# evolbioinfo/pastml

Hardware: AMD Instinct MI355X
Metric: ACR nodes*states*chars/sec (full marginal pass: P(t) + bottom-up + top-down + posteriors) (higher is better)
Workload: dtype f64; 1 GPU; BASELINE config 4 shard: balanced tree, 1048576 tips (2097151 nodes), k=64 states, F81, 32 characters per GPU (32 in total), marginal (BU+TD+posteriors); tips=1048576, nodes=2097151, states=64, chars_per_gpu=32, chars_total=32, substitution_model=F81, collective=local

## Files before the change

pastml_amd/csrc/pml_api.hip:

```cpp
#define PML_PLAIN_KERNELS
#include "pml_launch.h"
#include "pml_kernels_counts.h"
#include "pml_kernels_eigen_gemm.h"
#include "pml_comm.h"
#include "pml_pij_window.h"

#ifndef PML_BUILD_DIGEST
#define PML_BUILD_DIGEST "unknown"
#endif
static const char kBuildDigest[] = "PML_BUILD_DIGEST=" PML_BUILD_DIGEST;

static thread_local std::string g_last_error;

int pml_fail(int code, const char* fmt, ...) {
    char buf[1024];
    va_list ap;
    va_start(ap, fmt);
    vsnprintf(buf, sizeof(buf), fmt, ap);
    va_end(ap);
    g_last_error = buf;
    return code;
}

template <typename T>
// ... 973 lines not shown

static PmlSweepTraits sweep_traits(const pml_ctx* ctx) {
    PmlSweepTraits t;
    t.f81 = ctx->kind == PML_MODEL_F81;
    t.eigen_fused = eigen_fused(ctx);
    t.eigen_gemm = eigen_gemm(ctx);
    t.eigen_joint_valu = eigen_joint_valu(ctx);
    t.hky_fused = hky_fused(ctx);
    t.wide_states = wide_states(ctx);
    t.k = ctx->k;
    t.W = ctx->W;
    t.C = ctx->C;
    t.sched_cols = ctx->sched_cols;
    t.n_roots = ctx->n_roots;
    t.n_cherries = ctx->n_cherries;
    t.has_init = ctx->has_init;
    t.fuse = ctx->fuse;
    t.Gf = ctx->cols.Gf;
    t.Gt = ctx->cols.Gt;
    t.bu_wide_lanes = ctx->cols.bu_wide_lanes;
    t.level_lists_sorted = ctx->cols.level_lists_sorted;
    t.single_launch = single_launch_sweeps(ctx);
    t.blocks = block_schedule(ctx);
    t.super = super_sweeps(ctx);
    t.thin = thin_bottom_up(ctx);
    t.deep = deep_top_down(ctx);
    t.narrow_units = (int)ctx->tune.get(T_NARROW_UNITS, 0);
    t.no_td_tail = ctx->tune.on(T_NO_TD_TAIL);
    t.no_eigg_tiers = ctx->tune.on(T_NO_EIGG_TIERS);
    t.no_spin_wait = ctx->tune.on(T_NO_SPIN_WAIT);
    t.waves = PML_WAVES_PER_BLOCK;
    const int ks4 = (ctx->k + 3) / 4;
    t.eig_nb = ks4 % 4 == 0 ? 1 : (ks4 % 2 == 0 ? 2 : 4);
    return t;
}

static PmlSchedules schedules_of(const pml_ctx* ctx) {
    return {&ctx->blocks, &ctx->thin, &ctx->deep, &ctx->sup, &ctx->eig_tiers, &ctx->bt_tiers, &ctx->bu_level_vec_f,
            &ctx->bu_level_vec, &ctx->td_cherry_prefix};
}

static int run_plan(pml_ctx* ctx, const std::vector<PmlLaunch>& whole_plan, bool bottom_up, int is_marginal, bool force_prep) {
    const bool windowed = ctx->pij_window > 0 && ctx->kind == PML_MODEL_EIGEN;
    const int wtab = bottom_up ? 0 : 1;
    const std::vector<PmlWindowStep>* cached = nullptr;
    std::vector<PmlLaunch> cut;
    if (windowed) {
        auto same = [](const PmlLaunch& a, const PmlLaunch& b) {
            return a.op == b.op && a.list == b.list && a.kind == b.kind && a.bracket == b.bracket && a.branch == b.branch &&
                   a.signal == b.signal && a.cherries == b.cherries && a.first == b.first && a.count == b.count && a.arg == b.arg;
        };
        for (const pml_ctx::WindowCut& c : ctx->win_cuts)
            if (c.plan.size() == whole_plan.size() && std::equal(c.plan.begin(), c.plan.end(), whole_plan.begin(), same)) cached = &c.steps;
        if (cached == nullptr) {
            PmlWindowPlan W;
            const std::string bad = pml_plan_pij_window(whole_plan, ctx->forest, ctx->bu_order, ctx->td_parents, ctx->pij_window, W);
            if (!bad.empty()) return fail(PML_ERR_INVALID, "%s", bad.c_str());
            if (!W.branches.empty() && W.branches != ctx->win_branches[wtab])
                return fail(PML_ERR_INVALID, "the sweep's runs are not the ones the window's branch lists were uploaded for");
            if (ctx->win_cuts.size() >= 16) ctx->win_cuts.clear();
            ctx->win_cuts.push_back(pml_ctx::WindowCut{whole_plan, std::move(W.steps)});
            cached = &ctx->win_cuts.back().steps;
        }
        cut.reserve(cached->size());
        for (const PmlWindowStep& w : *cached) cut.push_back(w.launch);
    }
    static const std::vector<PmlWindowStep> no_steps;
    const std::vector<PmlWindowStep>& steps = windowed ? *cached : no_steps;
    const std::vector<PmlLaunch>& plan = windowed ? cut : whole_plan;
    size_t at = 0;
    const pml_ctx::EigenTiers& E = ctx->eig_tiers;
    const pml_ctx::BacktraceTiers& B = ctx->bt_tiers;
    const int* order = bottom_up ? ctx->d_bu_order : nullptr;
    const int* offsets = bottom_up ? ctx->d_bu_offsets : ctx->d_td_offsets;
    const int gemm_mode = bottom_up ? PML_EIGG_BU : PML_EIGG_TD;
    const int eig_mode = !bottom_up ? PML_EIG_TD : (is_marginal ? PML_EIG_BU_MARG : PML_EIG_BU_JOINT);
    int open = PML_NO_BRACKET;
    long long launches = 0;
    for (const PmlLaunch& r : plan) {
        if (ctx->tune.on(T_DEBUG))
            fprintf(stderr, "pml plan: branch %d op %d list %d kind %d first %d count %d arg %d bracket %d signal %d\n", r.branch,
                    r.op, r.list, r.kind, r.first, r.count, r.arg, r.bracket, (int)r.signal);
        if (r.bracket != open) {
            if (open != PML_NO_BRACKET) PML_TRY(prof_end(ctx, open, launches));
            if (r.bracket != PML_NO_BRACKET) PML_TRY(prof_begin(ctx));
            open = r.bracket;
            launches = 0;
        }
        ++launches;
        const PmlWindowStep* run = windowed ? &steps[at] : nullptr;
        ++at;
        if (run != nullptr && run->build_count > 0) {
            PML_TRY(launch_pij_wide_list(ctx, ctx->d_pij_window, ctx->pij_window, ctx->d_win_branches[wtab] + run->build_first,
                                         run->build_count));
            ++launches;
        }
        const bool joint = r.kind == EIG_JOINT, gemm = r.kind == EIG_GEMM;
        switch (r.op) {
            case OP_RESET_ERR:
                hipLaunchKernelGGL(reset_err_kernel, dim3((ctx->C + 63) / 64), dim3(64), 0, ctx->stream, ctx->d_err, ctx->C,
                                   r.arg ? ctx->d_tip_rest_count : nullptr);
                HIP_TRY(hipGetLastError());
                break;
            case OP_PREP:
                if (!windowed) PML_TRY(run_prep(ctx, force_prep, true));
                break;
            case OP_LOGLIK:
                hipLaunchKernelGGL(loglik_kernel, dim3((ctx->C + PML_BLOCK - 1) / PML_BLOCK), dim3(PML_BLOCK), 0, ctx->stream,
                                   tree_of(ctx), cols_of(ctx, true), state_of(ctx), ctx->C, is_marginal ? 1 : 0, ctx->h_loglik,
                                   ctx->h_err);
                HIP_TRY(hipGetLastError());
                break;
            case OP_LEVEL:
                PML_TRY(dispatch_sweep(ctx, (SweepKind)r.kind, r.list, r.first, r.count, r.cherries, bottom_up,
                                       windowed && (r.list == L_BU_PLAIN || r.list == L_TD_PLAIN) ? wtab : -1));
                break;
            case OP_ROOTS:
                PML_TRY(dispatch_sweep(ctx, SW_ROOTS, L_NONE, 0, r.count));
                break;
            case OP_LEVELS: {
                const bool whole = r.list == L_BU_FUSED || r.list == L_TD_FUSED;
                const int do_prep = (bottom_up && r.arg && (ctx->results.pij_stale() || force_prep)) ? 1 : 0;
                PML_TRY(dispatch_small_f81(ctx, bottom_up, r.signal, do_prep, whole ? r.first : 0, r.count,
                                           whole ? nullptr : ctx->d_unit_lists[r.list], whole ? nullptr : ctx->d_list_offsets[r.list] + r.first,
                                           bottom_up ? 0 : r.arg));
                break;
            }
            case OP_BLOCKS:
                PML_TRY(dispatch_blocks_f81(ctx, bottom_up, r.first, r.signal));
                break;
            case OP_SUPER:
                PML_TRY(dispatch_super_f81(ctx, bottom_up));
                break;
            case OP_STACK:
                PML_TRY(dispatch_stack_f81(ctx, bottom_up, r.first));
                break;
            case OP_EIG_TIPS:
                if (joint) PML_TRY(launch_eigen_joint_tips(ctx));
                else if (gemm) PML_TRY(launch_eigen_gemm(ctx, PML_EIGG_TIPS, ctx->d_tips, 0, ctx->n_tips));
                else PML_TRY(launch_eigen_tips(ctx, is_marginal ? 0 : 1));
                break;
            case OP_EIG_LEVEL: {
                const int* nodes = order ? order + r.first : nullptr;
                const int first = order ? 0 : r.first;
                if (joint) PML_TRY(launch_eigen_joint(ctx, ctx->d_bu_units + r.first, nullptr, 0, r.count));
                else if (gemm) PML_TRY(launch_eigen_gemm(ctx, gemm_mode, nodes, first, r.count));
                else PML_TRY(launch_eigen_fused(ctx, eig_mode, nodes, first, r.count, 0));
                break;
            }
            case OP_EIG_NARROW:
                if (joint) PML_TRY(launch_eigen_joint(ctx, ctx->d_bu_units, offsets, r.first, r.count));
                else if (gemm) PML_TRY(launch_eigen_gemm_narrow(ctx, gemm_mode, order, offsets, r.first, r.count));
                else PML_TRY(launch_eigen_narrow(ctx, eig_mode, order, offsets, r.first, r.count));
                break;
            case OP_EIG_TIER: {
                const pml_ctx::EigenTiers::Tier& T = E.tiers[r.first];
                if (joint) PML_TRY(launch_eigen_joint(ctx, E.d_units, E.d_lv, 0, T.depth, E.d_start + T.first_block, T.n_blocks));
                else PML_TRY(launch_eigen_gemm_narrow(ctx, PML_EIGG_BU, E.d_nodes, E.d_lv, 0, T.depth, E.d_start + T.first_block,
                                                      T.n_blocks));
                break;
            }
            case OP_BT_NARROW:
                hipLaunchKernelGGL(joint_backtrace_narrow_kernel, dim3(1, ctx->C), dim3(PML_BLOCK), 0, ctx->stream,
                                   tree_of(ctx), cols_of(ctx), state_of(ctx), ctx->d_td_offsets, r.first, r.count);
                HIP_TRY(hipGetLastError());
// ... 1457 lines not shown
```

pastml_amd/csrc/pml_kernels_f81.h:

```cpp
#pragma once
#include "pml_device.h"
#include "pml_schedule.h"

typedef unsigned char pml_jt;

struct PmlTree {
    int N;
    int n_roots;
    const int* parent;
    const int* first_child;
    const int* n_children;
    const double* dist;
    const int* post_rank;
    const unsigned char* kind;
};

struct PmlCols {
    int k, ks, W;
    int no_wide_lean;
    const u64* masks;
    const u64* masks_init;
    const double* pi;
    const double* active;
};
// ... 2327 lines not shown
        if (staged) td_stage_flush<G, R>(L, c, S, (stage & 4) != 0);
        cur = nxt;
        idx = nxt_idx;
    }
}


template <int G, int R>
__device__ __forceinline__ void td_f81_super_tips(const LaneCtx<G, R>& L, const PmlCols& c, const double (&prod3)[R],
                                                  i64 le, int cfc, const TipLane& tl, int jx) {
    constexpr int GC = Gather<G>::GC;
    double P3 = 0.0;
    bool have_P3 = false;
#pragma unroll
    for (int q = 0; q < 2; ++q) {
        const int ts = L.group_base + jx * GC + q;
        f81_finish_tip_word<G, R>(L, c, prod3, le, P3, have_P3, cfc + q, __shfl(tl.mask, ts, 64), __shfl(tl.e, ts, 64),
                                  __shfl(tl.s, ts, 64));
    }
}

template <int R>
struct TdSuperLoads {
    double po[R];
    double ls;
    i64 pe;
    double e, s;
    i64 be;
    u64 own;
    ChildLane cl;
    TipLane tl;
};

template <int G, int R>
__device__ __forceinline__ void td_f81_super_issue(const LaneCtx<G, R>& L, const PmlCols& c, const SuperRegs& s, int j,
                                                   TdSuperLoads<R>& ld) {
    const int ch = s.fc + j;
    node_load_vec<G, R>(L, c, L.post, s.n, ld.po);
    ld.ls = L.lhsum[s.n];
    ld.pe = L.lhe[s.n];
    ld.e = L.E[ch];
    ld.s = L.S[ch];
    ld.be = L.be[ch];
    ld.own = L.mask[(unsigned)ch];
    f81_gather_issue<G, R>(L, super_child<G>(s, j, L.g), ld.cl, ld.tl);
}

template <int R>
__device__ __forceinline__ void td_super_loads_arrived(TdSuperLoads<R>& ld) {
#pragma unroll
    for (int r = 0; r < R; ++r) asm volatile("" : "+v"(ld.po[r]));
    asm volatile("" : "+v"(ld.ls), "+v"(ld.pe), "+v"(ld.e), "+v"(ld.s), "+v"(ld.be), "+v"(ld.own));
    asm volatile("" : "+v"(ld.cl.e), "+v"(ld.cl.s), "+v"(ld.cl.mask), "+v"(ld.cl.be), "+v"(ld.tl.e), "+v"(ld.tl.s),
                      "+v"(ld.tl.mask));
}

template <int G, int R, bool LANES, bool PIPE>
__device__ __forceinline__ void td_f81_super_unit(const LaneCtx<G, R>& L, const PmlTree& t, const PmlCols& c,
                                                  const PmlState& st, const SuperRegs& s, int j, TdSuperLoads<R>& in,
                                                  double* ps_row) {
    if (PIPE) td_super_loads_arrived<R>(in);
    const u64 kbits = state_bits(c.k);
    const int ch = s.fc + j;
    const UnitRegs u = super_child<G>(s, j, L.g);
    double prod[R];
    const i64 pe = in.pe;
#pragma unroll
    for (int r = 0; r < R; ++r) prod[r] = in.po[r] * (in.ls * L.ipi_r[r]);
    const double e = in.e;
    const double s_child = in.s;
    const i64 bec = in.be;
    BuLoads<R> ld;
    ld.own = in.own;
// ... 217 lines not shown
    return bu_f81_marg_body<G, R, true, false>(L, t, c, st, un, top);
}

template <int G, int R>
__global__ void __launch_bounds__(PML_BLOCK) __attribute__((amdgpu_waves_per_eu(2, 2)))
bu_f81_stack_kernel(PmlTree t, PmlCols c, PmlState st, const PmlUnit* __restrict__ units, int n_level) {
    constexpr int UW = 64 / G;
    const int wave = threadIdx.x >> 6;
    const int sub = (threadIdx.x & 63) / G;
    LaneCtx<G, R> L;
    lane_ctx_init<G, R>(L, t, c, st);
    const int stride = gridDim.x * PML_WAVES_PER_BLOCK * UW;
    int idx = (blockIdx.x * PML_WAVES_PER_BLOCK + wave) * UW + sub;
    StackRegs cur = load_stack(units, idx < n_level ? idx : 0);
    for (int base = idx - sub; base < n_level; base += stride) {
        const int nxt_idx = idx + stride;
        const StackRegs nxt = load_stack(units, nxt_idx < n_level ? nxt_idx : 0);
        if (idx < n_level) {
            if (!bu_f81_stack_unit<G, R>(L, t, c, st, cur)) {
                bu_f81_unit_seq<G, R, false>(L, t, c, st, stack_child(cur, 0));
                bu_f81_unit_seq<G, R, false>(L, t, c, st, stack_child(cur, 1));
                __threadfence();
                UnitRegs un = stack_child(cur, 0);
                un.n = cur.n;
                un.fc = cur.fc;
                bu_f81_unit_seq<G, R, false>(L, t, c, st, un);
            }
        }
        cur = nxt;
        idx = nxt_idx;
    }
}

template <int G, int R>
__device__ __forceinline__ void td_f81_stack_unit(const LaneCtx<G, R>& L, const PmlTree& t, const PmlCols& c,
                                                  const PmlState& st, const StackRegs& s, int j) {
    const u64 kbits = state_bits(c.k);
    const int ch = s.fc + j;
    const int first = j ? s.g1 : s.g0;
    double prod[R];
    i64 pe;
    f81_parent_prod<G, R>(L, c, s.n, prod, pe);
    const double e = L.E[ch];
    const double s_child = L.S[ch];
    const i64 bec = L.be[ch];
    BuLoads<R> ld;
    stack_child_loads<G, R>(L, c, ch, first, ld);
    const u64 gmask = L.mask[(unsigned)(first + (L.g & 1))] & kbits;
    ld.own &= kbits;
    BuResult<R> v;
    double g0v[R], g1v[R];
#pragma unroll
    for (int r = 0; r < R; ++r) {
        g0v[r] = ld.v0[r];
        g1v[r] = ld.v1[r];
    }
    bu_f81_marg_body<G, R, true, false>(L, t, c, st, stack_child(s, j), ld, &v, false, true);
    double prod2[R];
    i64 pe2;
    {
        double mb[R], tdc[R], po[R], ls;
        const bool full = ld.own == kbits;
        if (!full) clean_word_to_vec<G, R>(L, c, ld.own, mb);
        i64 xe;
        f81_finish_child<G, R>(L, c, prod, pe, ch, e, s_child, bec, v.v, full, mb, tdc, xe, po, ls, pe2);
        if (st.td != nullptr) {
            node_store_vec<G, R>(L, c, L.td, ch, tdc);
            if (L.g == 0) L.te[ch] = xe;
        }
#pragma unroll
        for (int r = 0; r < R; ++r) prod2[r] = po[r] * (ls * L.ipi_r[r]);
    }
#pragma unroll
    for (int jx = 0; jx < 2; ++jx) {
        const int src = L.group_base + jx;
        const u64 word = __shfl(gmask, src, 64);
        double mb[R], tdc[R], po[R], ls;
        const bool full = word == kbits;
        if (!full) clean_word_to_vec<G, R>(L, c, word, mb);
        i64 xe, le;
        f81_finish_child<G, R>(L, c, prod2, pe2, first + jx, __shfl(ld.cl.e, src, 64), __shfl(ld.cl.s, src, 64),
                               __shfl(ld.cl.be, src, 64), jx ? g1v : g0v, full, mb, tdc, xe, po, ls, le);
        if (st.td != nullptr) {
            node_store_vec<G, R>(L, c, L.td, first + jx, tdc);
            if (L.g == 0) L.te[first + jx] = xe;
        }
    }
}

template <int G, int R>
__global__ void __launch_bounds__(PML_BLOCK)
td_f81_stack_kernel(PmlTree t, PmlCols c, PmlState st, const PmlUnit* __restrict__ units, int n_level) {
    constexpr int UW = 64 / G;
    const int wave = threadIdx.x >> 6;
    const int sub = (threadIdx.x & 63) / G;
    LaneCtx<G, R> L;
    lane_ctx_init<G, R>(L, t, c, st);
    const int n_units = 2 * n_level;
    const int stride = gridDim.x * PML_WAVES_PER_BLOCK * UW;
    int idx = (blockIdx.x * PML_WAVES_PER_BLOCK + wave) * UW + sub;
    StackRegs cur = load_stack(units, idx < n_units ? idx >> 1 : 0);
    for (int base = idx - sub; base < n_units; base += stride) {
        const int nxt_idx = idx + stride;
        const StackRegs nxt = load_stack(units, nxt_idx < n_units ? nxt_idx >> 1 : 0);
        if (idx < n_units) td_f81_stack_unit<G, R>(L, t, c, st, cur, idx & 1);
        cur = nxt;
        idx = nxt_idx;
    }
}


__device__ __forceinline__ double column_loglik(const PmlTree& t, const PmlCols& c, const PmlState& st, int col,
                                                int is_marginal) {
    const size_t colN = (size_t)col * t.N;
    double total = 0.0;
    for (int r = 0; r < t.n_roots; ++r) {
        const bool tip = t.n_children[r] == 0;
        const u64* m = c.masks + (colN + r) * c.W;
        double term;
        if (is_marginal) {
            term = 0.0;
            for (int s = 0; s < c.k; ++s) {
                const double b = tip ? (double)((m[s >> 6] >> (s & 63)) & 1ull) : st.bu[(colN + r) * c.ks + s];
                term += b * c.pi[(size_t)col * c.ks + s];
            }
        } else {
            term = -INFINITY;
            int arg = 0;
            for (int s = 0; s < c.k; ++s) {
                const double b = tip ? (double)((m[s >> 6] >> (s & 63)) & 1ull) : st.bu[(colN + r) * c.ks + s];
                const double v = b * c.pi[(size_t)col * c.ks + s];
                if (v > term) {
                    term = v;
                    arg = s;
                }
            }
            st.js[colN + r] = arg;
        }
        const double e2 = tip ? 0.0 : (double)st.be[colN + r];
        total += log(term) + e2 * 0.693147180559945309417232121458;
// ... 207 lines not shown
```

pastml_amd/csrc/pml_launch.h:

```cpp
#pragma once
#include "pml_host.h"
#include "pml_time_segments.h"

#define PML_GR_CASES(X)  \
    X(8, 4)              \
    X(1, 1)              \
    X(2, 1)              \
    X(4, 1)              \
    X(8, 1)              \
    X(16, 1)             \
    X(64, 1)             \
    X(32, 2)             \
    X(64, 2)             \
    X(64, 4)


#define PML_F81_CASES(X) \
    X(2, 2)              \
    X(4, 2)              \
    X(1, 1)              \
    X(1, 2)              \
    X(1, 4)              \
    X(2, 4)              \
    X(4, 4)              \
// ... 23 lines not shown
}

static bool thin_bottom_up(const pml_ctx* ctx) {
    return ctx->thin.ok && ctx->kind == PML_MODEL_F81 && !ctx->tune.on(T_NO_THIN) &&
           (ctx->cols.bu_shape().g < 8 || !ctx->tune.on(T_NO_THIN_WIDE));
}
static bool deep_top_down(const pml_ctx* ctx) {
    return ctx->deep.ok && ctx->kind == PML_MODEL_F81 && !ctx->tune.on(T_NO_THIN) && (ctx->cols.Gt < 8 || !ctx->tune.on(T_NO_THIN_WIDE));
}


static bool eigen_gemm(const pml_ctx* c) {
    const bool off = c->tune.on(T_NO_EIGEN_GEMM) || c->tune.on(T_NO_MFMA) || c->tune.on(T_NO_EIGEN_FUSED);
    if (off || !c->eig_fused_opt || c->kind != PML_MODEL_EIGEN || c->k < 2) return false;
    if (c->k <= 64) return c->W == 1;
    return c->k <= 128 && c->W == 2 && c->eig_sym_all && c->d_Asym != nullptr;
}


static bool eigen_joint_valu(const pml_ctx* c) {
    const bool off = c->tune.on(T_NO_EIGEN_JOINT_VALU);
    return !off && c->eigj_valu_opt && c->kind == PML_MODEL_EIGEN && c->k >= 2 && c->k <= 64 && c->W == 1 &&
           c->d_AinvT != nullptr;
}


PML_INTERNAL int dispatch_sweep_matrix(pml_ctx* ctx, SweepKind what, const int* level, int n_level, int window = -1);
PML_INTERNAL int dispatch_select(pml_ctx* ctx, int method, int force_joint, const u64* d_lh_mask);
PML_INTERNAL int dispatch_sweep_f81(pml_ctx* ctx, SweepKind what, const PmlUnit* units, int n_level, bool cherries, bool bu_sweep);
PML_INTERNAL int dispatch_sweep_f81_wide(pml_ctx* ctx, SweepKind what, const PmlUnit* units, int n_level, bool cherries, bool bu_sweep);
PML_INTERNAL int dispatch_small_f81(pml_ctx* ctx, bool bottom_up, bool signal, int do_prep, int first_level, int n_levels,
                                    const PmlUnit* units = nullptr, const int* d_offsets = nullptr, int skip_roots = 0);
PML_INTERNAL int dispatch_blocks_f81(pml_ctx* ctx, bool bottom_up, int which, bool signal);
PML_INTERNAL int dispatch_super_f81(pml_ctx* ctx, bool bottom_up);
PML_INTERNAL int dispatch_stack_f81(pml_ctx* ctx, bool bottom_up, int level);
PML_INTERNAL int launch_eigen_fused(pml_ctx* ctx, int mode, const int* nodes, int first, int n, int tips);
PML_INTERNAL int launch_eigen_narrow(pml_ctx* ctx, int mode, const int* nodes, const int* d_offsets, int first_level, int n_levels);
PML_INTERNAL int launch_eigen_tips(pml_ctx* ctx, int joint);
PML_INTERNAL int launch_pij_mfma(pml_ctx* ctx);
PML_INTERNAL int launch_pij_wide(pml_ctx* ctx);
PML_INTERNAL int launch_pij_wide_list(pml_ctx* ctx, double* window, long long B, const int* d_branches, int count, int col_begin = 0,
                                      int col_end = -1);
PML_INTERNAL int arm_pij_wide_list(pml_ctx* ctx);
PML_INTERNAL int launch_eigen_gemm(pml_ctx* ctx, int mode, const int* nodes, int first, int n);
PML_INTERNAL int launch_eigen_gemm_narrow(pml_ctx* ctx, int mode, const int* nodes, const int* d_offsets, int first_level,
                                          int n_levels, const int* d_blk_start = nullptr, int n_blocks = 1);
PML_INTERNAL int launch_eigen_gemm_wide(pml_ctx* ctx, int mode, const int* nodes, int first, int n);
PML_INTERNAL int launch_eigen_gemm_narrow_wide(pml_ctx* ctx, int mode, const int* nodes, const int* d_offsets, int first_level,
                                               int n_levels, const int* d_blk_start, int n_blocks);
PML_INTERNAL int launch_eigen_joint(pml_ctx* ctx, const PmlUnit* units, const int* d_offsets, int first, int n,
                                    const int* d_blk_start = nullptr, int n_blocks = 1);
PML_INTERNAL int launch_eigen_joint_tips(pml_ctx* ctx);
PML_INTERNAL int launch_pij_valu(pml_ctx* ctx);
PML_INTERNAL int launch_simulate(pml_ctx* ctx, int col, int rep_offset, u64 seed, void* d_states, size_t rs);
PML_INTERNAL int sim_frontier_depth(const pml_ctx* ctx, int n_tiles);
PML_INTERNAL int sim_subtree_lists(pml_ctx* ctx, int D);
static inline bool pij_windowed(const pml_ctx* ctx) {
    return ctx->pij_window > 0 && ctx->kind == PML_MODEL_EIGEN && ctx->d_pij_window != nullptr;
}
struct SimWindowDevice {
    PmlSimWindowPlan plan;
    std::vector<int4> lists;
    int* d_order = nullptr;
    int4* d_lists = nullptr;
    int* d_off = nullptr;
};
PML_INTERNAL int sim_window_prepare(pml_ctx* ctx, int D, CallScope& mem, SimWindowDevice& w);
// ... 83 lines not shown
```

pastml_amd/csrc/pml_launch_f81_super.hip:

```cpp
#include "pml_launch.h"

template <int G, int R, bool LANES, bool PIPE>
static void launch_td_super_f81(pml_ctx* ctx, dim3 grid, const PmlTree& t, const PmlCols& c, const PmlState& st) {
    hipLaunchKernelGGL((td_f81_super_kernel<G, R, LANES, PIPE>), grid, dim3(PML_BLOCK), 0, ctx->stream, t, c, st, ctx->sup.d_units,
                       ctx->sup.n);
}

template <int G, int R>
static void launch_super_f81(pml_ctx* ctx, bool bottom_up) {
    const PmlTree t = tree_of(ctx, true);
    const PmlCols c = cols_of(ctx, bottom_up);
    const PmlState st = state_of(ctx);
    const int upb = PML_WAVES_PER_BLOCK * (64 / G);
    const bool pipe = bottom_up || !ctx->tune.on(T_NO_TD_SUPER_PIPE);
    dim3 grid(grid_for(ctx, bottom_up ? ctx->sup.n : 2 * ctx->sup.n, upb, ctx->C, pipe), ctx->C), block(PML_BLOCK);
    const bool lanes = !ctx->tune.on(T_NO_TIP_LANES);
    if (bottom_up)
        hipLaunchKernelGGL((bu_f81_super_kernel<G, R>), grid, block, 0, ctx->stream, t, c, st, ctx->sup.d_units, ctx->sup.n);
    else if (pipe && lanes)
        launch_td_super_f81<G, R, true, true>(ctx, grid, t, c, st);
    else if (pipe)
        launch_td_super_f81<G, R, false, true>(ctx, grid, t, c, st);
    else if (lanes)
        launch_td_super_f81<G, R, true, false>(ctx, grid, t, c, st);
    else
        launch_td_super_f81<G, R, false, false>(ctx, grid, t, c, st);
}

template <int G, int R>
static void launch_stack_f81(pml_ctx* ctx, bool bottom_up, int a, int n) {
    const PmlTree t = tree_of(ctx, true);
    const PmlCols c = cols_of(ctx, bottom_up);
    const PmlState st = state_of(ctx);
    const int upb = PML_WAVES_PER_BLOCK * (64 / G);
    dim3 grid(grid_for(ctx, bottom_up ? n : 2 * n, upb, ctx->C), ctx->C), block(PML_BLOCK);
    if (bottom_up)
        hipLaunchKernelGGL((bu_f81_stack_kernel<G, R>), grid, block, 0, ctx->stream, t, c, st, ctx->sup.d_stack_bu + a, n);
    else
        hipLaunchKernelGGL((td_f81_stack_kernel<G, R>), grid, block, 0, ctx->stream, t, c, st, ctx->sup.d_stack_td + a, n);
}

int dispatch_super_f81(pml_ctx* ctx, bool bottom_up) {
    if (ctx->sup.n <= 0) return PML_OK;
    const auto [g, r] = ctx->cols.shape(bottom_up);
#define X(G_, R_)                                   \
    if (g == G_ && r == R_) {                       \
        launch_super_f81<G_, R_>(ctx, bottom_up);   \
        HIP_TRY(hipGetLastError());                 \
        return PML_OK;                              \
    }
    PML_SUPER_CASES(X)
#undef X
    return fail(PML_ERR_UNSUPPORTED, "no two-level F81 kernel for G=%d R=%d", g, r);
}

int dispatch_stack_f81(pml_ctx* ctx, bool bottom_up, int level) {
    const std::vector<int>& off = bottom_up ? ctx->sup.stack_bu_offsets : ctx->sup.stack_td_offsets;
    if (ctx->sup.n_stack == 0 || level + 1 >= (int)off.size()) return PML_OK;
    const int a = off[level], n = off[level + 1] - a;
    if (n <= 0) return PML_OK;
    const auto [g, r] = ctx->cols.shape(bottom_up);
#define X(G_, R_)                                         \
    if (g == G_ && r == R_) {                             \
        launch_stack_f81<G_, R_>(ctx, bottom_up, a, n);   \
        HIP_TRY(hipGetLastError());                       \
        return PML_OK;                                    \
    }
    PML_SUPER_CASES(X)
#undef X
    return fail(PML_ERR_UNSUPPORTED, "no stacked F81 kernel for G=%d R=%d", g, r);
}
```

pastml_amd/csrc/pml_schedule.cpp:

```cpp
#include "pml_schedule.h"
#include "pml_columns.h"

#include <algorithm>
#include <cstdarg>
#include <cstdio>

static std::string message(const char* fmt, ...) __attribute__((format(printf, 1, 2)));
static std::string message(const char* fmt, ...) {
    char buf[1024];
    va_list ap;
    va_start(ap, fmt);
    vsnprintf(buf, sizeof(buf), fmt, ap);
    va_end(ap);
    return buf;
}

std::string pml_check_tree(const PmlTreeArrays& t) {
    const int n_nodes = t.n_nodes, n_roots = t.n_roots, n_bu_levels = t.n_bu_levels, n_td_levels = t.n_td_levels;
    const int *parent = t.parent, *first_child = t.first_child, *n_children = t.n_children, *bu_offsets = t.bu_offsets,
              *bu_order = t.bu_order, *td_offsets = t.td_offsets, *td_parent_offsets = t.td_parent_offsets,
              *td_parents = t.td_parents, *post_rank = t.post_rank;
    if (n_nodes <= 0 || n_roots <= 0 || n_roots > n_nodes) return "bad node/root counts";
    if (!parent || !first_child || !n_children || !t.dist || !bu_offsets || !td_offsets || !td_parent_offsets || !post_rank)
        return "NULL tree array";
// ... 433 lines not shown
                   has_vec(fc[ch] + 1) && level_size(ch) <= 65536;
        };
        for (int n : order) {
            if (gone[n] || taken[n] || nch[n] != 2 || level_size(n) < stack_min || level_size(n) > 65536) continue;
            const int a = fc[n], b = a + 1;
            if (!plain2(a) || !plain2(b)) continue;
            stacked[n] = 1;
            taken[a] = taken[b] = novec[a] = novec[b] = 1;
            stack_list.push_back(n);
        }
    }
    if (!tune.on(T_STACK_MIN) && (long long)stack_list.size() * 3 * 2 < (long long)n_stored - 3 * (long long)sup_list.size())
        stack_list.clear();
    std::vector<int> stack_children, sup_children;
    for (int n : stack_list) {
        gone[n] = gone[fc[n]] = gone[fc[n] + 1] = 1;
        stack_children.push_back(fc[n]);
        stack_children.push_back(fc[n] + 1);
    }
    if (!stack_list.empty()) {
        const std::vector<int> depth_of = node_depths(f);
        U.stack_bu_offsets.assign(max_h + 1, 0);
        for (int n : stack_list) ++U.stack_bu_offsets[fh[n]];
        for (int l = 0; l < max_h; ++l) U.stack_bu_offsets[l + 1] += U.stack_bu_offsets[l];
        std::vector<int> by_depth(stack_list);
        std::stable_sort(by_depth.begin(), by_depth.end(), [&](int x, int y) { return depth_of[x] < depth_of[y]; });
        U.stack_td_offsets.assign(n_td_levels + 1, 0);
        for (int n : by_depth) ++U.stack_td_offsets[depth_of[n] + 1];
        for (int l = 0; l < n_td_levels; ++l) U.stack_td_offsets[l + 1] += U.stack_td_offsets[l];
        P.sup.stack_bu = describe(f, stack_list);
        P.sup.stack_td = describe(f, by_depth);
        P.sup.stack_children = describe(f, stack_children);
        U.n_stack = (int)stack_list.size();
        if (tune.on(T_DEBUG)) fprintf(stderr, "pastml_hip: %d stacked units\n", U.n_stack);
    }
    if (sup_list.empty() && stack_list.empty()) return;
    std::vector<int> bu_r, td_r;
    U.bu_offsets_r.assign(1, 0);
    for (int l = 0; l < max_h; ++l) {
        for (int q = off[l]; q < off[l + 1]; ++q)
            if (!gone[order[q]]) bu_r.push_back(order[q]);
        U.bu_offsets_r.push_back((int)bu_r.size());
    }
    U.td_offsets_r.assign(1, 0);
    for (int l = 0; l < n_td_levels; ++l) {
        for (int q = f.td_parent_offsets_f[l]; q < f.td_parent_offsets_f[l + 1]; ++q)
            if (!gone[f.tdp[q]]) td_r.push_back(f.tdp[q]);
        U.td_offsets_r.push_back((int)td_r.size());
    }
    for (int n : sup_list) {
        sup_children.push_back(fc[n]);
        sup_children.push_back(fc[n] + 1);
    }
    U.n_child_units = (int)sup_children.size();
    P.sup.child_units = describe(f, sup_children);
    P.sup.bu_units_r = describe(f, bu_r);
    P.sup.td_units_r = describe(f, td_r);
    U.bu_level_vec_r = stored_child01_levels(P.sup.bu_units_r, U.bu_offsets_r.data(), max_h);
    P.sup.bu_units_r.resize(bu_r.size() + 1, P.sup.units[0]);
    P.sup.td_units_r.resize(td_r.size() + 1, P.sup.units[0]);
    if (P.shape_sort) {
        P.sup.bu_units_rs = units_by_shape(P.sup.bu_units_r, U.bu_offsets_r, bu_r.size());
        P.sup.td_units_rs = units_by_shape(P.sup.td_units_r, U.td_offsets_r, td_r.size(), f.shape_ordered ? fh.data() : nullptr);
    }
    P.sup.lists = true;
    U.n = (int)sup_list.size();
    U.ok = U.n > 0 || U.n_stack >= 64 || (U.n_stack > 0 && tune.on(T_STACK_MIN));
// ... 386 lines not shown
}

std::vector<PmlLaunch> pml_plan_top_down(const PmlForest& f, const PmlSchedules& s, const PmlSweepTraits& t, bool wants_signal) {
    const int nd = (int)f.td_offsets.size() - 1;
    const bool td_small = t.single_launch && t.f81;
    const bool levels_f81 = t.f81 && !td_small;
    const bool signal = wants_signal && t.C <= 64 && !t.no_spin_wait;
    Plan p;
    auto roots = [&](int list, int head) {
        if (head == 0) p.add(OP_ROOTS, L_NONE, 0, t.n_roots);
        else p.add(OP_LEVELS, list, 0, head);
        p.bracket = 1;
    };
    if (levels_f81 && t.blocks) {
        const PmlBlockSchedule& B = *s.blocks;
        p.branch = TD_BLOCKS;
        const int head = t.n_roots <= 64 ? narrow_levels(t, B.top_td_offsets, nd, true, t.C) : 0;
        roots(L_TOP_TD, head);
        p.levels(OP_LEVEL, L_TOP_TD, B.top_td_offsets, head, nd, false, td_fused_kind);
        p.add(OP_BLOCKS, L_NONE, 0, B.n_blocks).signal = signal;
        return p.v;
    }
    if (levels_f81 && t.super) {
        const PmlSuperSchedule& U = *s.sup;
        p.branch = TD_SUPER;
        int head = t.n_roots <= 64 ? narrow_levels(t, U.td_offsets_r, nd, true, t.C) : 0;
        for (int l = 0; l < nd && U.n_stack > 0; ++l)
            if (U.stack_td_offsets[l + 1] > U.stack_td_offsets[l]) {
                head = std::min(head, l);
                break;
            }
        if (head < 2) head = 0;
        roots(L_REST_TD, head);
        p.levels(OP_LEVEL, t.level_lists_sorted ? L_REST_TD_SORTED : L_REST_TD, U.td_offsets_r, head, nd, false, td_fused_kind,
                 [&](int l) { add_stack(p, U, U.stack_td_offsets, l); });
        p.bracket = 3;
        if (U.n > 0) p.add(OP_SUPER, L_NONE, 0, U.n);
        return p.v;
    }
    const int head = (levels_f81 && t.n_roots <= 64) ? narrow_levels(t, f.td_parent_offsets_f, nd, true, t.C) : 0;
    const bool deep = levels_f81 && t.deep && s.deep->first_depth > head;
    p.branch = td_small ? TD_ONE_LAUNCH : deep ? TD_DEEP : t.eigen_gemm ? TD_GEMM : t.eigen_fused ? TD_EIG_FUSED : TD_LEVELS;
    if (td_small) p.bracket = 1;
    else roots(L_TD_FUSED, head);
    if (td_small) p.add(OP_LEVELS, L_TD_FUSED, 0, nd).signal = signal;
    else if (t.eigen_gemm) eigen_top_down(p, f, t, EIG_GEMM, 2 * t.waves * 16);
    else if (t.eigen_fused) eigen_top_down(p, f, t, EIG_FUSED, t.waves * t.eig_nb);
    if (p.branch != TD_LEVELS && p.branch != TD_DEEP) return p.v;
    const int fused_list = t.level_lists_sorted ? L_TD_FUSED_SORTED : L_TD_FUSED;
    auto hint = [&](size_t from) {
        const std::vector<int>& pre = *s.td_cherry_prefix;
        for (size_t i = from; i < p.v.size(); ++i) {
            const size_t a = (size_t)p.v[i].first, b = a + (size_t)p.v[i].count;
            if (!pre.empty() && b < pre.size()) p.v[i].cherries = pre[b] != pre[a];
        }
    };
    const size_t from = p.v.size();
    if (deep) {
        p.levels(OP_LEVEL, fused_list, f.td_parent_offsets_f, head, s.deep->first_depth, false, td_fused_kind);
        hint(from);
        p.add(OP_BLOCKS, L_NONE, 1, s.deep->n_blocks);
        return p.v;
    }
    int tail = 0;
    if (t.f81 && t.Gt < 8 && !t.no_td_tail) {
        tail = std::min(nd - head, narrow_levels(t, f.td_parent_offsets_f, nd, false, t.C, 0, 1));
        if (tail < 2) tail = 0;
    }
    if (t.f81) {
        p.levels(OP_LEVEL, fused_list, f.td_parent_offsets_f, head, nd - tail, false, td_fused_kind);
// ... 34 lines not shown
```

pastml_amd/csrc/pml_schedule.h:

```cpp
#pragma once
#include <cstdlib>
#include <string>
#include <vector>

#define PML_KIND_TIP 0
#define PML_KIND_CHERRY 1
#define PML_KIND_STORED 2

struct __attribute__((aligned(32))) PmlUnit {
    int n, fc, packed, pad;
    int cfc[4];
};

#define PML_PACKED_TWO_STORED ((1 << 11) | (1 << 8) | (3 << 4) | 2)

#define PML_SMALL_BLOCK 512

#define PML_TUNABLES(X)                                                                                              \
    X(GRID_CAP, 0, 0) X(SMALL_MANY_NODES, 0, 0) X(BLOCK_MAX_WORK, 0, 0)    \
    X(NO_MFMA, 1, 0) X(NO_EIGEN_FUSED, 1, 0) X(NO_HKY_FUSED, 1, 0)      \
    X(BLOCK_THREADS, 0, 0) X(EIG_BLOCKS, 0, 0) X(NO_EIGEN_GEMM, 1, 0) X(NO_EIGEN_JOINT_VALU, 1, 0) X(EIGJ_BLOCKS, 0, 0) \
    X(EIGJ_TIP_BLOCKS, 0, 0) X(EIGJ_ONE_TIPS_KERNEL, 1, 0) X(EIGJ_TIER_THIN, 0, 1) X(EIGJ_TIER_DEPTH, 0, 1)            \
    X(NO_EIGJ_TIERS, 1, 1) X(NO_BT_TIERS, 1, 1) X(NO_SHAPE_SORT, 1, 1) X(NO_SUPER, 1, 1) X(SUPER_MIN, 0, 1)            \
    X(STACK_MIN, 0, 1) X(NO_STACK, 1, 1) X(DEBUG, 1, 0) X(BLOCK_NODES, 0, 1) X(BLOCK_MAX_STORED, 0, 1)                 \
    X(BLOCK_HEIGHT_CAP, 0, 1) X(SMALL_MAX_NODES, 0, 1) X(F81_R, 0, 1) X(F81_TD_R, 0, 1) X(NO_GRAPH, 1, 1)              \
    X(NARROW_UNITS, 0, 0) X(NO_EIGG_TIERS, 1, 0) X(NO_SPIN_WAIT, 1, 0)   \
    X(PIJ_STAGE_ROWS, 0, 0) X(PIJ_BLOCKS, 0, 0) X(NO_HEIGHT_ORDER, 1, 1) X(NO_TD_TAIL, 1, 0) X(NO_PIJ_VALU, 1, 0) X(PIJ_VALU, 1, 0) X(NO_PIJ_WIDE, 1, 0) X(NO_EIGJ_PIPE, 1, 0) \
    X(THIN_UNITS, 0, 1) X(THIN_BYTES, 0, 1) X(THIN_BLOCK_NODES, 0, 1) X(NO_THIN, 1, 0) X(NO_THIN_WIDE, 1, 0) X(BU_WIDE, 0, 1) X(SORT_LEVELS, 0, 1) X(NO_WIDE_LEAN, 1, 0) X(SHAPE_ORDER, 0, 1) \
    X(PARS_MAX_COLS, 0, 0) X(PARS_THIN, 0, 0) X(COMPRESS_MAX_COLS, 0, 0) X(COMPRESS_PLAIN_ATOMICS, 1, 0) \
    X(PIJ_WINDOW, 0, 0) X(NO_KEEP_TIP_ROWS, 1, 0) X(NO_TIP_LANES, 1, 0) X(NO_TD_SUPER_PIPE, 1, 0)
enum PmlTunable {
#define X(name, flag, tree) T_##name,
    PML_TUNABLES(X)
#undef X
    T_COUNT
};
static const char* const kTunableName[T_COUNT] = {
#define X(name, flag, tree) #name,
    PML_TUNABLES(X)
#undef X
};
static const bool kTunableFlag[T_COUNT] = {
#define X(name, flag, tree) flag != 0,
    PML_TUNABLES(X)
#undef X
};
static const bool kTunableTree[T_COUNT] = {
#define X(name, flag, tree) tree != 0,
    PML_TUNABLES(X)
#undef X
};
struct PmlTune {
    long long val[T_COUNT];
    bool has[T_COUNT];
    PmlTune() {
        for (int i = 0; i < T_COUNT; ++i) {
            const std::string var = std::string("PASTML_HIP_") + kTunableName[i];
            const char* e = getenv(var.c_str());
            has[i] = e != nullptr;
            val[i] = e ? atoll(e) : 0;
        }
    }
    bool on(int i) const { return has[i]; }
// ... 8 lines not shown
    int *d_bu_start = nullptr, *d_bu_levels = nullptr, *d_bu_lv = nullptr;
    int *d_td_start = nullptr, *d_td_levels = nullptr, *d_td_lv = nullptr;
    PmlUnit *d_top_bu_units = nullptr, *d_top_td_units = nullptr;
    int *d_top_bu_offsets = nullptr, *d_top_td_offsets = nullptr;
    std::vector<int> top_bu_offsets, top_td_offsets;
    std::vector<char> top_bu_vec;
};
struct PmlThinSchedule {
    bool ok = false;
    int floor_level = 0;
    int top_level = 0;
    struct Tier { int first_block, n_blocks; };
    std::vector<Tier> tiers;
    PmlUnit* d_units = nullptr;
    int *d_start = nullptr, *d_levels = nullptr, *d_lv = nullptr;
};
struct PmlDeepSchedule {
    bool ok = false;
    int first_depth = 0, n_blocks = 0;
    PmlUnit* d_units = nullptr;
    int *d_start = nullptr, *d_levels = nullptr, *d_lv = nullptr;
};
struct PmlSuperSchedule {
    bool ok = false;
    int n = 0;
    PmlUnit* d_units = nullptr;
    PmlUnit* d_child_units = nullptr;
    PmlUnit *d_bu_units_r = nullptr, *d_td_units_r = nullptr;
    PmlUnit *d_bu_units_rs = nullptr, *d_td_units_rs = nullptr;
    int n_child_units = 0;
    int n_stack = 0;
    PmlUnit *d_stack_bu = nullptr, *d_stack_td = nullptr, *d_stack_children = nullptr;
    std::vector<int> stack_bu_offsets, stack_td_offsets;
    int *d_bu_offsets_r = nullptr, *d_td_offsets_r = nullptr;
    std::vector<int> bu_offsets_r, td_offsets_r;
    std::vector<char> bu_level_vec_r;
};
struct PmlEigenTiers {
    bool ok = false;
    int first_level = 0;
    int top_level = 0;
    struct Tier { int first_block, n_blocks, depth; };
    std::vector<Tier> tiers;
    PmlUnit* d_units = nullptr;
    int *d_lv = nullptr, *d_start = nullptr;
    int* d_nodes = nullptr;
    int widest = 0;
};
struct PmlBacktraceTiers {
    bool ok = false;
    int first_depth = 0;
    struct Tier { int first_block, n_blocks, depth; };
    std::vector<Tier> tiers;
    int *d_nodes = nullptr, *d_lv = nullptr, *d_start = nullptr;
};

struct PmlTreeArrays {
    int n_nodes, n_roots, n_bu_levels, n_td_levels;
    const int *parent, *first_child, *n_children, *bu_offsets, *bu_order, *td_offsets, *td_parent_offsets, *td_parents,
        *post_rank;
    const double* dist;
};

struct PmlNumbering {
    std::vector<int> old_of_new, new_of_old;
    std::vector<int> parent, first_child, n_children, bu_order, td_parents, post_rank;
// ... 105 lines not shown
};
#define PML_NO_BRACKET 255
struct PmlLaunch {
    unsigned char op, list, kind;
    unsigned char bracket;
    unsigned char branch;
    bool signal;
    bool cherries;
    int first, count;
    int arg;
};
struct PmlSweepOutcome {
    int n_signals = 0;
    bool final_signals = false;
    bool has_params = false;
    bool fused_joint = false;
    void then(const PmlSweepOutcome& next) {
        n_signals += next.n_signals;
        final_signals = next.final_signals;
        has_params = has_params || next.has_params;
        fused_joint = fused_joint || next.fused_joint;
    }
};
struct PmlSweepTraits {
    bool f81, eigen_fused, eigen_gemm, eigen_joint_valu, hky_fused, wide_states;
    int k, W, C, sched_cols, n_roots, n_cherries;
    bool has_init, fuse;
    int Gf, Gt;
    bool bu_wide_lanes, level_lists_sorted;
    bool single_launch, blocks, super, thin, deep;
    int narrow_units;
    bool no_td_tail, no_eigg_tiers, no_spin_wait;
    int waves, eig_nb;
};
struct PmlSchedules {
    const PmlBlockSchedule* blocks;
    const PmlThinSchedule* thin;
    const PmlDeepSchedule* deep;
    const PmlSuperSchedule* sup;
    const PmlEigenTiers* eig;
    const PmlBacktraceTiers* bt;
    const std::vector<char>*bu_level_vec_f, *bu_level_vec;
    const std::vector<int>* td_cherry_prefix;
};

#define PML_PLAN __attribute__((visibility("hidden")))
PML_PLAN std::string pml_check_tree(const PmlTreeArrays& t);
PML_PLAN PmlForest pml_plan_forest(PmlTreeArrays& t, const PmlTune& tune, bool fuse, PmlNumbering& num);
PML_PLAN PmlTreePlan pml_plan_tree(const PmlForest& f, const PmlTreeArrays& t, const PmlTune& tune);
PML_PLAN PmlThinPlan pml_plan_thin_ends(const PmlForest& f, const PmlTune& tune, int thin);
PML_PLAN std::vector<PmlLaunch> pml_plan_bottom_up(const PmlForest& f, const PmlSchedules& s, const PmlSweepTraits& t, bool is_marginal);
PML_PLAN std::vector<PmlLaunch> pml_plan_top_down(const PmlForest& f, const PmlSchedules& s, const PmlSweepTraits& t, bool wants_signal);
PML_PLAN std::vector<PmlLaunch> pml_plan_backtrace(const PmlForest& f, const PmlSchedules& s, const PmlSweepTraits& t, int* head);
PML_PLAN PmlSweepOutcome pml_plan_outcome(const std::vector<PmlLaunch>& plan);
```

Baseline: 609.3 billion node*state*char/s.

## Chain deepest stacked top-down level into the super kernel via LDS rows

```diff
diff --git a/pastml_amd/csrc/pml_api.hip b/pastml_amd/csrc/pml_api.hip
--- a/pastml_amd/csrc/pml_api.hip
+++ b/pastml_amd/csrc/pml_api.hip
@@ -1029,6 +1029,7 @@
     t.waves = PML_WAVES_PER_BLOCK;
     const int ks4 = (ctx->k + 3) / 4;
     t.eig_nb = ks4 % 4 == 0 ? 1 : (ks4 % 2 == 0 ? 2 : 4);
+    t.td_chain = t.f81 && t.super && ctx->sup.chain_depth >= 0 && !ctx->tune.on(T_NO_TD_CHAIN) && !ctx->tune.on(T_NO_TD_SUPER_PIPE);
     return t;
 }
 
@@ -1076,8 +1077,9 @@
     long long launches = 0;
     for (const PmlLaunch& r : plan) {
         if (ctx->tune.on(T_DEBUG))
-            fprintf(stderr, "pml plan: branch %d op %d list %d kind %d first %d count %d arg %d bracket %d signal %d\n", r.branch,
-                    r.op, r.list, r.kind, r.first, r.count, r.arg, r.bracket, (int)r.signal);
+            fprintf(stderr, "pml plan: branch %d op %d list %d kind %d first %d count %d arg %d bracket %d signal %d%s\n", r.branch,
+                    r.op, r.list, r.kind, r.first, r.count, r.arg, r.bracket, (int)r.signal,
+                    r.op == OP_SUPER && !bottom_up && r.arg > 0 ? " (chained: with the stacked units of depth arg - 1)" : "");
         if (r.bracket != open) {
             if (open != PML_NO_BRACKET) PML_TRY(prof_end(ctx, open, launches));
             if (r.bracket != PML_NO_BRACKET) PML_TRY(prof_begin(ctx));
@@ -1127,7 +1129,7 @@
                 PML_TRY(dispatch_blocks_f81(ctx, bottom_up, r.first, r.signal));
                 break;
             case OP_SUPER:
-                PML_TRY(dispatch_super_f81(ctx, bottom_up));
+                PML_TRY(dispatch_super_f81(ctx, bottom_up, bottom_up ? -1 : r.arg - 1));
                 break;
             case OP_STACK:
                 PML_TRY(dispatch_stack_f81(ctx, bottom_up, r.first));
diff --git a/pastml_amd/csrc/pml_kernels_f81.h b/pastml_amd/csrc/pml_kernels_f81.h
--- a/pastml_amd/csrc/pml_kernels_f81.h
+++ b/pastml_amd/csrc/pml_kernels_f81.h
@@ -2383,13 +2383,15 @@
     TipLane tl;
 };
 
-template <int G, int R>
+template <int G, int R, bool ROW = true>
 __device__ __forceinline__ void td_f81_super_issue(const LaneCtx<G, R>& L, const PmlCols& c, const SuperRegs& s, int j,
                                                    TdSuperLoads<R>& ld) {
     const int ch = s.fc + j;
-    node_load_vec<G, R>(L, c, L.post, s.n, ld.po);
-    ld.ls = L.lhsum[s.n];
-    ld.pe = L.lhe[s.n];
+    if (ROW) {
+        node_load_vec<G, R>(L, c, L.post, s.n, ld.po);
+        ld.ls = L.lhsum[s.n];
+        ld.pe = L.lhe[s.n];
+    }
     ld.e = L.E[ch];
     ld.s = L.S[ch];
     ld.be = L.be[ch];
@@ -2673,9 +2675,45 @@
     }
 }
 
-template <int G, int R>
+struct TdRowNowhere {
+    template <int G, int R>
+    __device__ __forceinline__ void operator()(const LaneCtx<G, R>&, const PmlCols&, int, const double (&)[R], double, i64) const {}
+};
+#define PML_TD_CHAIN_SLOT(G, R) ((G) * (R) + 2)
+struct TdRowToLds {
+    double* slots;
+    template <int G, int R>
+    __device__ __forceinline__ void operator()(const LaneCtx<G, R>& L, const PmlCols& c, int jx, const double (&po)[R], double ls,
+                                               i64 le) const {
+        double* row = slots + jx * PML_TD_CHAIN_SLOT(G, R);
+#pragma unroll
+        for (int r = 0; r < R; r += 2) {
+            double2 t2;
+            t2.x = L.st(r) < c.ks ? po[r] : 0.0;
+            t2.y = L.st(r) < c.ks ? po[r + 1] : 0.0;
+            *reinterpret_cast<double2*>(row + L.st(r)) = t2;
+        }
+        if (L.g == 0) {
+            row[G * R] = ls;
+            *reinterpret_cast<i64*>(row + G * R + 1) = le;
+        }
+    }
+};
+template <int G, int R>
+__device__ __forceinline__ void td_chain_row_load(const LaneCtx<G, R>& L, const double* row, TdSuperLoads<R>& ld) {
+#pragma unroll
+    for (int r = 0; r < R; r += 2) {
+        const double2 t2 = *reinterpret_cast<const double2*>(row + L.st(r));
+        ld.po[r] = t2.x;
+        ld.po[r + 1] = t2.y;
+    }
+    ld.ls = row[G * R];
+    ld.pe = *reinterpret_cast<const i64*>(row + G * R + 1);
+}
+
+template <int G, int R, class RowSink = TdRowNowhere>
 __device__ __forceinline__ void td_f81_stack_unit(const LaneCtx<G, R>& L, const PmlTree& t, const PmlCols& c,
-                                                  const PmlState& st, const StackRegs& s, int j) {
+                                                  const PmlState& st, const StackRegs& s, int j, const RowSink& sink = RowSink()) {
     const u64 kbits = state_bits(c.k);
     const int ch = s.fc + j;
     const int first = j ? s.g1 : s.g0;
@@ -2722,6 +2760,7 @@
         i64 xe, le;
         f81_finish_child<G, R>(L, c, prod2, pe2, first + jx, __shfl(ld.cl.e, src, 64), __shfl(ld.cl.s, src, 64),
                                __shfl(ld.cl.be, src, 64), jx ? g1v : g0v, full, mb, tdc, xe, po, ls, le);
+        sink(L, c, jx, po, ls, le);
         if (st.td != nullptr) {
             node_store_vec<G, R>(L, c, L.td, first + jx, tdc);
             if (L.g == 0) L.te[first + jx] = xe;
@@ -2747,6 +2786,75 @@
         if (idx < n_units) td_f81_stack_unit<G, R>(L, t, c, st, cur, idx & 1);
         cur = nxt;
         idx = nxt_idx;
+    }
+}
+
+template <int G, int R, bool LANES>
+__global__ void __launch_bounds__(PML_BLOCK) __attribute__((amdgpu_waves_per_eu(R == 8 ? 2 : 1, R == 8 ? 2 : 8)))
+td_f81_chain_kernel(PmlTree t, PmlCols c, PmlState st, const PmlUnit* __restrict__ units, int n_level,
+                    const PmlUnit* __restrict__ stack_units) {
+    constexpr int UW = 64 / G, SLOT = PML_TD_CHAIN_SLOT(G, R);
+    const int wave = threadIdx.x >> 6;
+    const int sub = (threadIdx.x & 63) / G;
+    __shared__ __attribute__((aligned(16))) double tip_rows[LANES ? PML_BLOCK * R : 2];
+    __shared__ __attribute__((aligned(16))) double node_rows[PML_WAVES_PER_BLOCK * 2 * UW * SLOT];
+    double* const ps_row = LANES ? tip_rows + (wave * UW + sub) * (G * R) : nullptr;
+    double* const wave_rows = node_rows + wave * (2 * UW * SLOT);
+    LaneCtx<G, R> L;
+    lane_ctx_init<G, R>(L, t, c, st);
+    const int n_units = 2 * n_level;
+    const int n_stack_units = n_level / 2;
+    const int n_tiles = (n_stack_units + UW - 1) / UW;
+    const int stride = gridDim.x * PML_WAVES_PER_BLOCK;
+    const int j = sub & 1;
+    const TdRowToLds sink = {wave_rows + 2 * sub * SLOT};
+    auto stack_desc = [&](int q) {
+        const int i = q * UW + sub;
+        return load_stack(stack_units, i < n_stack_units ? i >> 1 : 0);
+    };
+    auto super_desc = [&](int q, int p) {
+        const int i = (4 * q + p) * UW + sub;
+        return load_super(units, i < n_units ? i >> 1 : 0);
+    };
+    auto pass = [&](int q, int p, const SuperRegs& s, TdSuperLoads<R>& ld) {
+        td_chain_row_load<G, R>(L, wave_rows + ((p * UW + sub) >> 1) * SLOT, ld);
+        if ((4 * q + p) * UW + sub < n_units) td_f81_super_unit<G, R, LANES, true>(L, t, c, st, s, j, ld, ps_row);
+    };
+    int q = blockIdx.x * PML_WAVES_PER_BLOCK + wave;
+    StackRegs sk = stack_desc(q);
+    SuperRegs ua = super_desc(q, 0), ub = super_desc(q, 1);
+    TdSuperLoads<R> la, lb;
+    td_f81_super_issue<G, R, false>(L, c, ua, j, la);
+    for (; q < n_tiles; q += stride) {
+        const StackRegs sk_next = stack_desc(q + stride);
+        if (q * UW + sub < n_stack_units) td_f81_stack_unit<G, R>(L, t, c, st, sk, j, sink);
+        wave_sync_lds();
+        {
+            const SuperRegs un = super_desc(q, 2);
+            td_f81_super_issue<G, R, false>(L, c, ub, j, lb);
+            pass(q, 0, ua, la);
+            ua = un;
+        }
+        {
+            const SuperRegs un = super_desc(q, 3);
+            td_f81_super_issue<G, R, false>(L, c, ua, j, la);
+            pass(q, 1, ub, lb);
+            ub = un;
+        }
+        {
+            const SuperRegs un = super_desc(q + stride, 0);
+            td_f81_super_issue<G, R, false>(L, c, ub, j, lb);
+            pass(q, 2, ua, la);
+            ua = un;
+        }
+        {
+            const SuperRegs un = super_desc(q + stride, 1);
+            td_f81_super_issue<G, R, false>(L, c, ua, j, la);
+            pass(q, 3, ub, lb);
+            ub = un;
+        }
+        wave_sync_lds();
+        sk = sk_next;
     }
 }
 
diff --git a/pastml_amd/csrc/pml_launch.h b/pastml_amd/csrc/pml_launch.h
--- a/pastml_amd/csrc/pml_launch.h
+++ b/pastml_amd/csrc/pml_launch.h
@@ -79,7 +79,7 @@
 PML_INTERNAL int dispatch_small_f81(pml_ctx* ctx, bool bottom_up, bool signal, int do_prep, int first_level, int n_levels,
                                     const PmlUnit* units = nullptr, const int* d_offsets = nullptr, int skip_roots = 0);
 PML_INTERNAL int dispatch_blocks_f81(pml_ctx* ctx, bool bottom_up, int which, bool signal);
-PML_INTERNAL int dispatch_super_f81(pml_ctx* ctx, bool bottom_up);
+PML_INTERNAL int dispatch_super_f81(pml_ctx* ctx, bool bottom_up, int chain_depth = -1);
 PML_INTERNAL int dispatch_stack_f81(pml_ctx* ctx, bool bottom_up, int level);
 PML_INTERNAL int launch_eigen_fused(pml_ctx* ctx, int mode, const int* nodes, int first, int n, int tips);
 PML_INTERNAL int launch_eigen_narrow(pml_ctx* ctx, int mode, const int* nodes, const int* d_offsets, int first_level, int n_levels);
diff --git a/pastml_amd/csrc/pml_launch_f81_super.hip b/pastml_amd/csrc/pml_launch_f81_super.hip
--- a/pastml_amd/csrc/pml_launch_f81_super.hip
+++ b/pastml_amd/csrc/pml_launch_f81_super.hip
@@ -7,10 +7,23 @@
 }
 
 template <int G, int R>
-static void launch_super_f81(pml_ctx* ctx, bool bottom_up) {
+static void launch_td_chain_f81(pml_ctx* ctx, int a, const PmlTree& t, const PmlCols& c, const PmlState& st) {
+    const int tiles = (2 * ctx->sup.n + 4 * (64 / G) - 1) / (4 * (64 / G));
+    dim3 grid(grid_for(ctx, tiles, PML_WAVES_PER_BLOCK, ctx->C, true), ctx->C);
+    if (!ctx->tune.on(T_NO_TIP_LANES))
+        hipLaunchKernelGGL((td_f81_chain_kernel<G, R, true>), grid, dim3(PML_BLOCK), 0, ctx->stream, t, c, st, ctx->sup.d_units,
+                           ctx->sup.n, ctx->sup.d_stack_td + a);
+    else
+        hipLaunchKernelGGL((td_f81_chain_kernel<G, R, false>), grid, dim3(PML_BLOCK), 0, ctx->stream, t, c, st, ctx->sup.d_units,
+                           ctx->sup.n, ctx->sup.d_stack_td + a);
+}
+
+template <int G, int R>
+static void launch_super_f81(pml_ctx* ctx, bool bottom_up, int chain_first) {
     const PmlTree t = tree_of(ctx, true);
     const PmlCols c = cols_of(ctx, bottom_up);
     const PmlState st = state_of(ctx);
+    if (chain_first >= 0) return launch_td_chain_f81<G, R>(ctx, chain_first, t, c, st);
     const int upb = PML_WAVES_PER_BLOCK * (64 / G);
     const bool pipe = bottom_up || !ctx->tune.on(T_NO_TD_SUPER_PIPE);
     dim3 grid(grid_for(ctx, bottom_up ? ctx->sup.n : 2 * ctx->sup.n, upb, ctx->C, pipe), ctx->C), block(PML_BLOCK);
@@ -40,14 +53,22 @@
         hipLaunchKernelGGL((td_f81_stack_kernel<G, R>), grid, block, 0, ctx->stream, t, c, st, ctx->sup.d_stack_td + a, n);
 }
 
-int dispatch_super_f81(pml_ctx* ctx, bool bottom_up) {
+int dispatch_super_f81(pml_ctx* ctx, bool bottom_up, int chain_depth) {
     if (ctx->sup.n <= 0) return PML_OK;
+    int chain_first = -1;
+    if (chain_depth >= 0) {
+        const std::vector<int>& off = ctx->sup.stack_td_offsets;
+        if (bottom_up || chain_depth != ctx->sup.chain_depth || chain_depth + 1 >= (int)off.size() ||
+            (long long)(off[chain_depth + 1] - off[chain_depth]) * 4 != ctx->sup.n)
+            return fail(PML_ERR_INVALID, "no chained two-level launch for depth %d", chain_depth);
+        chain_first = off[chain_depth];
+    }
     const auto [g, r] = ctx->cols.shape(bottom_up);
-#define X(G_, R_)                                   \
-    if (g == G_ && r == R_) {                       \
-        launch_super_f81<G_, R_>(ctx, bottom_up);   \
-        HIP_TRY(hipGetLastError());                 \
-        return PML_OK;                              \
+#define X(G_, R_)                                                \
+    if (g == G_ && r == R_) {                                    \
+        launch_super_f81<G_, R_>(ctx, bottom_up, chain_first);   \
+        HIP_TRY(hipGetLastError());                              \
+        return PML_OK;                                           \
     }
     PML_SUPER_CASES(X)
 #undef X
diff --git a/pastml_amd/csrc/pml_schedule.cpp b/pastml_amd/csrc/pml_schedule.cpp
--- a/pastml_amd/csrc/pml_schedule.cpp
+++ b/pastml_amd/csrc/pml_schedule.cpp
@@ -489,7 +489,17 @@
         P.sup.stack_td = describe(f, by_depth);
         P.sup.stack_children = describe(f, stack_children);
         U.n_stack = (int)stack_list.size();
-        if (tune.on(T_DEBUG)) fprintf(stderr, "pastml_hip: %d stacked units\n", U.n_stack);
+        int deepest = n_td_levels - 1;
+        while (deepest >= 0 && U.stack_td_offsets[deepest + 1] == U.stack_td_offsets[deepest]) --deepest;
+        const int a = U.stack_td_offsets[deepest], cnt = U.stack_td_offsets[deepest + 1] - a;
+        bool lined_up = (long long)cnt * 4 == (long long)sup_list.size();
+        for (int m = 0; m < cnt && lined_up; ++m) {
+            const int n = by_depth[a + m], g0 = fc[fc[n]], g1 = fc[fc[n] + 1];
+            lined_up = sup_list[4 * m] == g0 && sup_list[4 * m + 1] == g0 + 1 && sup_list[4 * m + 2] == g1 &&
+                       sup_list[4 * m + 3] == g1 + 1;
+        }
+        if (lined_up) U.chain_depth = deepest;
+        if (tune.on(T_DEBUG)) fprintf(stderr, "pastml_hip: %d stacked units, chain depth %d\n", U.n_stack, U.chain_depth);
     }
     if (sup_list.empty() && stack_list.empty()) return;
     std::vector<int> bu_r, td_r;
@@ -942,10 +952,11 @@
             }
         if (head < 2) head = 0;
         roots(L_REST_TD, head);
+        const int chained = t.td_chain && U.n > 0 ? U.chain_depth : -1;
         p.levels(OP_LEVEL, t.level_lists_sorted ? L_REST_TD_SORTED : L_REST_TD, U.td_offsets_r, head, nd, false, td_fused_kind,
-                 [&](int l) { add_stack(p, U, U.stack_td_offsets, l); });
+                 [&](int l) { if (l != chained) add_stack(p, U, U.stack_td_offsets, l); });
         p.bracket = 3;
-        if (U.n > 0) p.add(OP_SUPER, L_NONE, 0, U.n);
+        if (U.n > 0) p.add(OP_SUPER, L_NONE, 0, U.n).arg = chained + 1;
         return p.v;
     }
     const int head = (levels_f81 && t.n_roots <= 64) ? narrow_levels(t, f.td_parent_offsets_f, nd, true, t.C) : 0;
diff --git a/pastml_amd/csrc/pml_schedule.h b/pastml_amd/csrc/pml_schedule.h
--- a/pastml_amd/csrc/pml_schedule.h
+++ b/pastml_amd/csrc/pml_schedule.h
@@ -28,7 +28,7 @@
     X(PIJ_STAGE_ROWS, 0, 0) X(PIJ_BLOCKS, 0, 0) X(NO_HEIGHT_ORDER, 1, 1) X(NO_TD_TAIL, 1, 0) X(NO_PIJ_VALU, 1, 0) X(PIJ_VALU, 1, 0) X(NO_PIJ_WIDE, 1, 0) X(NO_EIGJ_PIPE, 1, 0) \
     X(THIN_UNITS, 0, 1) X(THIN_BYTES, 0, 1) X(THIN_BLOCK_NODES, 0, 1) X(NO_THIN, 1, 0) X(NO_THIN_WIDE, 1, 0) X(BU_WIDE, 0, 1) X(SORT_LEVELS, 0, 1) X(NO_WIDE_LEAN, 1, 0) X(SHAPE_ORDER, 0, 1) \
     X(PARS_MAX_COLS, 0, 0) X(PARS_THIN, 0, 0) X(COMPRESS_MAX_COLS, 0, 0) X(COMPRESS_PLAIN_ATOMICS, 1, 0) \
-    X(PIJ_WINDOW, 0, 0) X(NO_KEEP_TIP_ROWS, 1, 0) X(NO_TIP_LANES, 1, 0) X(NO_TD_SUPER_PIPE, 1, 0)
+    X(PIJ_WINDOW, 0, 0) X(NO_KEEP_TIP_ROWS, 1, 0) X(NO_TIP_LANES, 1, 0) X(NO_TD_SUPER_PIPE, 1, 0) X(NO_TD_CHAIN, 1, 0)
 enum PmlTunable {
 #define X(name, flag, tree) T_##name,
     PML_TUNABLES(X)
@@ -103,6 +103,7 @@
     int n_stack = 0;
     PmlUnit *d_stack_bu = nullptr, *d_stack_td = nullptr, *d_stack_children = nullptr;
     std::vector<int> stack_bu_offsets, stack_td_offsets;
+    int chain_depth = -1;
     int *d_bu_offsets_r = nullptr, *d_td_offsets_r = nullptr;
     std::vector<int> bu_offsets_r, td_offsets_r;
     std::vector<char> bu_level_vec_r;
@@ -274,6 +275,7 @@
     int narrow_units;
     bool no_td_tail, no_eigg_tiers, no_spin_wait;
     int waves, eig_nb;
+    bool td_chain;
 };
 struct PmlSchedules {
     const PmlBlockSchedule* blocks;
```

Result: faster. 634.9 billion node*state*char/s, median of 6 (+4.2%).
